# aurelienwaite/SparkNet

Measured on AMD Instinct MI355X. Metric: images/sec AlexNet training (227x227) at 1/2/4/8 MI355X; scaling efficiency, higher is better.
Workload: dtype bf16; 1 GPU; model=caffenet (bvlc_reference_caffenet / AlexNet), global_batch=256, per_gpu_batch=256, parallelism=dp1, algorithm=local SGD, tau=50, RCCL all-reduce weight averaging, hipgraph=True, streams=3, feed_group=2, fused_input_fold=True, fp8_layers=0, fp8_wgrad=False

## Files before the change

### sparknet_amd/ops/hip.py

```python
from __future__ import annotations

import contextlib
import ctypes as C
import dataclasses
import os
from typing import NamedTuple

import torch

from . import _lib
from ..utils import features
from .gemm import (EPI_BF16, EPI_F32, EPI_F32_ACC, ConvGeom, Dense, FlipW, Fp8Side, Im2col, colsum, fp8_side_output,
                   gemm, linear_dgrad, linear_fwd, linear_wgrad, side_bytes)
from .spec import POOL_MAX, ConvNdSpec, ConvSpec, PoolSpec

call = _lib.call
BF16 = torch.bfloat16
DGRAD_INPLACE_WEIGHTS = False


def _c(t: torch.Tensor) -> torch.Tensor:
    return t if t.is_contiguous() else t.contiguous()


# ... 1 lines not shown
    if t.is_contiguous():
        return t.shape[-1]
    if t.dim() != 4 or t.stride(-1) != 1:
        return 0
    N, H, W, Cc = t.shape
    ld = t.stride(2)
    if ld < Cc or t.stride(1) != W * ld or (N > 1 and t.stride(0) != H * W * ld):
        return 0
    return ld


def as_bf16(t: torch.Tensor | None) -> torch.Tensor | None:
    if t is None:
        return None
    t = _c(t)
    if t.dtype == BF16:
        return t
    if t.dtype != torch.float32:
        raise TypeError(f"GPU activations are bf16 or fp32, got {t.dtype}")
    out = torch.empty(t.shape, dtype=BF16, device=t.device)
    call("cast_f32_bf16", t, out, t.numel())
    return out


def _round8(n: int) -> int:
    return -(-n // 8) * 8



def _implicit_ok(s: ConvSpec) -> bool:
    return s.Cg % 8 == 0 and s.C % 8 == 0


def _unit_conv(s: ConvSpec) -> bool:
    return s.sh == 1 and s.sw == 1 and s.dh == 1 and s.dw == 1


def _wgrad_implicit_ok(s: ConvSpec) -> bool:
    return _implicit_ok(s) and s.Kg % 8 == 0


def _dgrad_flip_geom_ok(s: ConvSpec) -> bool:
    return _unit_conv(s) and _wgrad_implicit_ok(s)


def _plain_window(s: ConvSpec, r: int, p: int) -> bool:
    return s.groups == 1 and _unit_conv(s) and s.R == s.S == r and s.ph == s.pw == p


def _tile_rows_fit(s: ConvSpec, extra: int, lds_bytes: int) -> bool:
    return min(s.H, (191 + s.Q - 1) // s.Q + extra) * s.W * s.C * 2 <= lds_bytes


def _weight_kpad(w: torch.Tensor, s: ConvSpec) -> tuple[torch.Tensor, int]:
    kred = s.R * s.S * s.Cg
    kpad = _round8(kred)
    w2 = w.reshape(s.K, kred)
    if kpad == kred:
        return _c(w2), kpad
    out = torch.zeros((s.K, kpad), dtype=BF16, device=w.device)
    out[:, :kred].copy_(w2)
    return out, kpad


def _im2col(x: torch.Tensor, s: ConvSpec, g: int, kpad: int) -> torch.Tensor:
    M = s.N * s.P * s.Q
    col = torch.empty((M, kpad), dtype=BF16, device=x.device)
    call("im2col", x, col, s.N, s.H, s.W, s.C, s.P, s.Q, s.R, s.S, s.sh, s.sw, s.ph, s.pw, s.dh, s.dw,
         s.Cg, kpad, g * s.Cg)
    return col


def _geom(s: ConvSpec, ldx: int | None = None) -> ConvGeom:
    return ConvGeom(s.N, s.H, s.W, s.C if ldx is None else ldx, s.P, s.Q, s.R, s.S, s.sh, s.sw, s.ph, s.pw, s.dh, s.dw, s.Cg)


def _s2d_plan(s: ConvSpec):
    if _implicit_ok(s) or s.groups != 1 or s.sh != s.sw or s.dh != 1 or s.dw != 1:
        return None
    f = s.sh
    cp = s.C
    while (f * f * cp) % 8:
        cp += 1
    rf, sf = -(-s.R // f), -(-s.S // f)
    hs, ws = s.P + rf - 1, s.Q + sf - 1
    s2 = ConvSpec(s.N, hs, ws, f * f * cp, s.K, rf, sf, 1, 1, 0, 0, 1, 1, 1)
    assert s2.P == s.P and s2.Q == s.Q
    return f, cp, rf, sf, s2


def _s2d_input(x, s: ConvSpec, plan):
    f, cp, rf, sf, s2 = plan
    x2 = torch.empty((s.N, s2.H, s2.W, s2.C), dtype=BF16, device=x.device)
    call("s2d_input", x, x2, s.N, s.H, s.W, s.C, s2.H, s2.W, f, cp, s.ph, s.pw)
    return x2


def _s2d_cached(entry, x):
    return entry[2] if entry is not None and entry[:2] == (x.data_ptr(), x._version) else None


def _slice_ok(s: ConvSpec) -> bool:
    return s.groups == 1 and _wgrad_implicit_ok(s)


_MAX_PIX = 1 << 24


def _image_chunk(s: ConvSpec) -> int:
    per = max(s.H * s.W, s.P * s.Q, 1)
    plan = _s2d_plan(s)
    if plan is not None:
        per = max(per, plan[4].H * plan[4].W)
    return s.N if s.N * per < _MAX_PIX else max(1, (_MAX_PIX - 1) // per)


def conv_forward(x, w, b, s: ConvSpec, relu=False, ws=None, folded=None, out=None):
    nb = _image_chunk(s)
    if nb < s.N:
        y = out if out is not None else torch.empty((s.N, s.P, s.Q, s.K), dtype=BF16, device=x.device)
        for n0 in range(0, s.N, nb):
            n1 = min(s.N, n0 + nb)
            conv_forward(x[n0:n1], w, b, s.with_batch(n1 - n0), relu, None,
                         folded[n0:n1] if folded is not None else None, out=y[n0:n1])
        if ws is not None and folded is not None:
            ws.s2d_full = (x.data_ptr(), x._version, folded)
        return y
    ldx = chan_stride(x)
    if not (ldx and _slice_ok(s)):
        x, ldx = _c(x), s.C
    assert x.dtype == BF16 and w.dtype == BF16, (x.dtype, w.dtype)
    if out is not None:
        ldo = chan_stride(out)
        assert (out.is_contiguous() or _slice_ok(s)) and ldo and tuple(out.shape) == (s.N, s.P, s.Q, s.K) \
            and out.dtype == BF16, "conv output slice needs an ungrouped implicit conv and an NHWC channel-slice view"
    plan = _s2d_plan(s)
    if plan is not None:
        f, cp, rf, sf, s2 = plan
        w2 = ws.w2 if ws is not None else None
        if w2 is None:
            w2 = torch.empty((s.K, rf, sf, s2.C), dtype=BF16, device=x.device)
            call("s2d_weight", _c(w), w2, s.K, s.R, s.S, s.C, f, cp, rf, sf)
        else:
            assert tuple(w2.shape) == (s.K, rf, sf, s2.C) and w2.dtype == BF16 and w2.is_contiguous()
        x2 = folded if folded is not None else _s2d_input(x, s, plan)
        if ws is not None:
            ws.s2d = (x.data_ptr(), x._version, x2)
        return conv_forward(x2, w2, b, s2, relu, out=out)
    M = s.N * s.P * s.Q
    if out is not None:
        y, ldy = out, chan_stride(out)
    else:
        y, ldy = torch.empty((s.N, s.P, s.Q, s.K), dtype=BF16, device=x.device), s.K
    if ldx == s.C and ldy == s.K and x.is_contiguous() and packed3x3k64_ok(s):
        from . import gemm as G
        side = G._SIDE if _side_covers(y) else None
        if side is None or not side.e5m2:
            q = (None, None, None)
            if side is not None:
                q = (side.q.data_ptr() + (y.data_ptr() - side.base.data_ptr()) // 2, side.slot, side.part)
                side.launches += 1
            call("conv_packed3x3k64", x, _c(w), b, y, s.N, s.H, s.W, s.C, s.K, int(relu), *q)
            return y
    direct_io = ldx == s.C and ldy == s.K and x.is_contiguous() and not _side_covers(y)
    if direct_io and packed_conv_ok(s):
        call("conv_packed3x3", x, _c(w), b, y, s.N, s.H, s.W, s.C, s.K, int(relu))
        return y
    if direct_io and packed11_conv_ok(s):
        call("conv_packed1x1", x, _c(w), b, y, s.N, s.H, s.W, s.C, s.K, int(relu))
        return y
    if direct_io and packed44_conv_ok(s):
        call("conv_packed4x4", x, _c(w), b, y, s.N, s.H, s.W, s.C, s.K, int(relu))
        return y
    if direct_io and direct_conv_ok(s):
        call("conv3x3_direct", x, _c(w), b, None, y, s.N, s.H, s.W, s.C, s.K, s.ph, int(relu), 0)
        return y
    if direct_io and direct96_split_ok(s):
        wc = _c(w)
        for j in range(0, s.K, 96):
            call("conv3x3_direct", x, wc[j:j + 96], b[j:j + 96] if b is not None else None, None, y[..., j:],
                 s.N, s.H, s.W, s.C, 96, s.ph, int(relu), s.K)
        return y
    if direct_io and ldy == s.K and depthwise_ok(s) and _dw_io_ok(x, w, y):
        call("conv_dw_fwd", x, w, b, y, s.N, s.H, s.W, s.C, s.sh, s.sw, s.ph, s.pw, int(relu))
        return y
    if direct_io and ldy == s.K and grouped_ok(s) and _dw_io_ok(x, w, y):
        call(GROUPED_FWD, x, w, b, y, s.N, s.H, s.W, s.C, s.Cg, s.sh, s.sw, s.ph, s.pw, int(relu))
        return y
    if _implicit_ok(s):
        kred = s.R * s.S * s.Cg
        A = Im2col(x, _geom(s, ldx), kcontig=True, gstride=s.Cg)
        B = Dense(_c(w.reshape(s.K, kred)), kred, True, gstride=s.Kg * kred)
        gemm(M, s.Kg, kred, A, B, y, ldy, epi=EPI_BF16, groups=s.groups, c_gstride=s.Kg, bias=b, relu=relu)
        return y
    assert ldy == s.K, "explicit im2col path writes contiguous outputs"
    wp, kpad = _weight_kpad(w, s)
    y2 = y.view(M, s.K)
    for g in range(s.groups):
        col = _im2col(x, s, g, kpad)
        wg = wp[g * s.Kg:(g + 1) * s.Kg]
        bg = b[g * s.Kg:(g + 1) * s.Kg] if b is not None else None
        gemm(M, s.Kg, kpad, Dense(col, kpad, True), Dense(_c(wg), kpad, True), y2[:, g * s.Kg:], s.K,
             epi=EPI_BF16, bias=bg, relu=relu)
    return y


_DIRECT_C64 = features.enabled("conv_direct_c64")
_DIRECT_K96 = features.enabled("conv_direct_k96")


def direct_c64_ok(s: ConvSpec) -> bool:
    return _DIRECT_C64 and s.C == 64 and s.K == 64 and _plain_window(s, 3, 1)


def direct_conv_ok(s: ConvSpec) -> bool:
    return direct_c64_ok(s) or (_DIRECT_K96 and s.C == 48 and s.K == 96 and _plain_window(s, 3, 0))


_DIRECT96 = features.enabled("conv_direct96")


def direct96_split_ok(s: ConvSpec) -> bool:
    return _DIRECT96 and 0 < s.C <= 64 and s.C % 8 == 0 and s.K > 96 and s.K % 96 == 0 and _plain_window(s, 3, 1)


_PACKED11 = features.enabled("conv_packed11")


def packed11_conv_ok(s: ConvSpec) -> bool:
    return (_PACKED11 and 0 < s.C <= 64 and s.C % 8 == 0 and s.K == 64 and _plain_window(s, 1, 0)
            and _tile_rows_fit(s, 1, 36864))


_PACKED = features.enabled("conv_packed")


def packed_conv_ok(s: ConvSpec) -> bool:
    return (_PACKED and s.K == 96 and 0 < s.C <= 48 and s.C % 8 == 0 and _plain_window(s, 3, 0) and s.Q > 0
            and _tile_rows_fit(s, 3, 38400) and s.P * s.Q * 96 < 2 ** 31)


_PACKED44 = features.enabled("conv_packed44")


def packed44_conv_ok(s: ConvSpec) -> bool:
    return (_PACKED44 and s.K == 64 and s.C in (8, 16) and _plain_window(s, 4, 0) and s.Q > 0
            and _tile_rows_fit(s, 4, 22528) and s.P * s.Q * 64 < 2 ** 31)


_PACKED_K64 = features.enabled("conv_packed_k64")


def packed3x3k64_ok(s: ConvSpec) -> bool:
    return (_PACKED_K64 and s.K == 64 and s.C == 8 and _plain_window(s, 3, 0) and s.Q > 0
            and _tile_rows_fit(s, 3, 16384) and s.P * s.Q * 64 < 2 ** 31)


_DIRECT_FP8 = features.enabled("conv_direct_fp8")


def direct_fp8_ok(s: ConvSpec) -> bool:
    return _DIRECT_FP8 and direct_c64_ok(s)


def depthwise_ok(s: ConvSpec) -> bool:
    return (s.groups == s.C == s.K and s.C % 8 == 0 and s.R == 3 and s.S == 3 and s.dh == 1 and s.dw == 1
            and features.enabled("conv_depthwise"))


def _dw_io_ok(*tensors) -> bool:
    return all(t is None or (t.dtype == BF16 and t.is_contiguous() and t.data_ptr() % 16 == 0) for t in tensors)


def _dw_part(s: ConvSpec, device) -> tuple[torch.Tensor, int]:
    k = _lib.kernels()
    k.sn_conv_dw_part_floats.restype = C.c_longlong
    n = int(k.sn_conv_dw_part_floats(*(C.c_longlong(v) for v in (s.N, s.P, s.Q, s.C))))
    if n <= 0:
        raise ValueError(f"depthwise weight gradient: unsupported geometry {s}")
    return torch.empty(n, dtype=torch.float32, device=device), n


GROUPED_WIDTHS = (4, 8, 16)
_GROUPED_MAX_PIX = 1 << 30
GROUPED_FWD, GROUPED_WGRAD, GROUPED_DGRAD = "conv_grouped_fwd", "conv_grouped_wgrad", "conv_grouped_dgrad"


def grouped_ok(s: ConvSpec) -> bool:
    return (1 < s.Cg == s.Kg and s.Cg in GROUPED_WIDTHS and s.C % 16 == 0 and s.R == 3 and s.S == 3
            and s.dh == 1 and s.dw == 1 and s.sh in (1, 2) and s.sw in (1, 2)
            and max(s.N * s.H * s.W, s.N * s.P * s.Q) < _GROUPED_MAX_PIX and s.P > 0 and s.Q > 0
            and max(s.C, s.ph, s.pw) <= 1 << 20 and features.enabled("conv_grouped"))


def _grouped_part(s: ConvSpec, device) -> tuple[torch.Tensor, int]:
    k = _lib.kernels()
    k.sn_conv_grouped_part_floats.restype = C.c_longlong
    n = int(k.sn_conv_grouped_part_floats(*(C.c_longlong(v) for v in (s.N, s.P, s.Q, s.C, s.Cg))))
    if n <= 0:
        raise ValueError(f"grouped weight gradient: unsupported geometry {s}")
    return torch.empty(n, dtype=torch.float32, device=device), n


def _side_covers(t: torch.Tensor) -> bool:
    from . import gemm as G
    return G._SIDE is not None and G._SIDE.covers(t)


def dgrad_uses_flip(s: ConvSpec) -> bool:
    return _dgrad_flip_geom_ok(s) and not DGRAD_INPLACE_WEIGHTS


class Fp8Dgrad(NamedTuple):
    scales: object
    dy_slot: int
    wt_slot: int
    dy_side: object = None

    @property
    def dy_only(self) -> bool:
        return bool(getattr(self.dy_side, "only", False))


class Fp8Wgrad(NamedTuple):
    scales: object
    x_slot: int
    xq: torch.Tensor
    dy_slot: int


@dataclasses.dataclass
class ConvScratch:
    s2d: tuple | None = None
    s2d_full: tuple | None = None
    wt: torch.Tensor | None = None
    w2: torch.Tensor | None = None
    dw2: torch.Tensor | None = None
    fp8_dgrad: Fp8Dgrad | None = None
    fp8_wgrad: Fp8Wgrad | None = None
    fp8_dx_side: tuple | None = None
    fp8_dx_side_out: object = None

    def release(self) -> None:
        self.__init__()


class FlipBatch:

    def __init__(self, items, device):
        self.items = list(items)
        self.device = torch.device(device)
        self._build()

    def _ptrs(self):
        return [(w.data_ptr(), wt.data_ptr()) for w, wt, *_ in self.items]

    def _build(self):
        lib = _lib.kernels()
        lib.sn_flip_desc_size.restype = C.c_int
        size = lib.sn_flip_desc_size()
        buf = (C.c_char * (size * len(self.items)))()
        for i, (w, wt, G, Kg, R, S, Cg) in enumerate(self.items):
            assert w.is_contiguous() and wt.is_contiguous() and w.dtype == BF16 and wt.dtype == BF16
            assert w.numel() == wt.numel() == G * Kg * R * S * Cg < (1 << 31)
            lib.sn_flip_desc(C.byref(buf, i * size), C.c_void_p(w.data_ptr()), C.c_void_p(wt.data_ptr()),
                             *(C.c_longlong(v) for v in (G, Kg, R, S, Cg)))
        self.descs = torch.frombuffer(bytearray(buf), dtype=torch.uint8).to(self.device)
        self.max_tiles = max(G * R * S * -(-Kg // 64) * -(-Cg // 64) for _, _, G, Kg, R, S, Cg in self.items)
        self.ptrs = self._ptrs()

    def run(self) -> None:
        if self._ptrs() != self.ptrs:
            self._build()
        call("flip_weights_multi", self.descs, len(self.items), self.max_tiles)


def _pad_cols(t2: torch.Tensor, n: int) -> torch.Tensor:
    out = torch.zeros((t2.shape[0], n), dtype=t2.dtype, device=t2.device)
    out[:, :t2.shape[1]].copy_(t2)
    return out


def conv_backward(dy, x, w, s: ConvSpec, need_dx: bool, dw=None, db=None, gate=None, ws=None,
                  dw_acc=True, db_acc=True, dx_out=None):
    ws = ConvScratch() if ws is None else ws
    nb = _image_chunk(s)
    if dx_out is not None and need_dx and chan_stride(dx_out) != s.C and not (
            _dgrad_flip_geom_ok(s) and chan_stride(dx_out) and nb >= s.N
            and ws.fp8_dgrad is None and ws.fp8_dx_side is None):
        dx_out.copy_(conv_backward(dy, x, w, s, need_dx, dw, db, gate, ws, dw_acc, db_acc))
        return dx_out
    dx, side = dx_out if need_dx else None, None
    side_req, ws.fp8_dx_side = ws.fp8_dx_side, None
    if side_req is not None and need_dx and dx_out is None:
        dx = torch.empty((s.N, s.H, s.W, s.C), dtype=BF16, device=x.device)
        side = Fp8Side(dx, *side_req)
    with fp8_side_output(side) if side is not None else contextlib.nullcontext():
        if nb >= s.N:
            out = _conv_backward(dy, x, w, s, need_dx, dw, db, gate, ws, None, dw_acc, db_acc, dx)
        else:
            if dx is None and need_dx:
                dx = torch.empty((s.N, s.H, s.W, s.C), dtype=BF16, device=x.device)
            out = dx
            full = _s2d_cached(ws.s2d_full, x)
            dyq = _fp8_dyq(dy, ws)
            f8w = ws.fp8_wgrad
            for n0 in range(0, s.N, nb):
                n1 = min(s.N, n0 + nb)
                cws = ConvScratch(wt=ws.wt, fp8_dgrad=ws.fp8_dgrad,
                                  fp8_wgrad=f8w and f8w._replace(xq=f8w.xq[n0:n1]),
                                  s2d=full if full is None else (x[n0:n1].data_ptr(), x._version, full[n0:n1]))
                _conv_backward(dy[n0:n1], x[n0:n1], w, s.with_batch(n1 - n0), need_dx, dw, db,
                               gate[n0:n1] if gate is not None else None, cws,
                               None if dyq is None else dyq[n0:n1], dw_acc, db_acc, dx[n0:n1] if need_dx else None)
                dw_acc = db_acc = True
    ws.fp8_dx_side_out = side if out is dx else None
    return out


def _conv_backward(dy, x, w, s: ConvSpec, need_dx, dw, db, gate, ws: ConvScratch, dyq, dw_acc, db_acc, dx_out):
    kred = s.R * s.S * s.Cg
    plan = _s2d_plan(s) if s.Kg % 8 == 0 else None
    ldd, ldx = chan_stride(dy), chan_stride(x)
    if plan is not None or not _slice_ok(s) or not (ldd and ldx):
        dy, ldd, x, ldx = _c(dy), s.K, _c(x), s.C
    M = s.N * s.P * s.Q
    dy2 = dy.view(M, s.K) if ldd == s.K else dy
    fused_db = db is not None and dw is not None and (plan is not None or _wgrad_implicit_ok(s))
    f8w = ws.fp8_wgrad
    if (f8w is not None and dw is not None and plan is None and ldd == s.K and ldx == s.C
            and fp8_wgrad_ok(s) and f8w.xq.shape[0] == s.N):
        if dyq is None:
            dyq = _fp8_dyq(dy, ws)
        _conv_wgrad_fp8(dy2, dyq, s, M, kred, f8w, dw, db, dw_acc, db_acc, _dy_fp8_only(ws))
        dw, db, fused_db = None, None, False
    if (dw is not None or db is not None) and _dy_fp8_only(ws):
        _no_bf16_dy("a bf16 weight / bias gradient")
    _conv_wgrad(dy2, x, s, M, kred, plan, fused_db, dw, db, ws, dw_acc, db_acc, ldd, ldx)
    return _conv_dgrad(dy, x, w, s, M, gate, ws, dyq, ldd, ldx, dx_out) if need_dx else None


def _conv_wgrad(dy2, x, s, M, kred, plan, fused_db, dw, db, ws, dw_acc, db_acc, ldd, ldx):
    if ((dw is not None or db is not None) and plan is None and ldd == s.K and ldx == s.C and depthwise_ok(s)
            and _dw_io_ok(dy2, x)):
        part, n = _dw_part(s, x.device)
        call("conv_dw_wgrad", dy2, x, part, n, dw, 0 if dw is None else 1 + int(dw_acc),
             db, 0 if db is None else 1 + int(db_acc), s.N, s.H, s.W, s.C, s.sh, s.sw, s.ph, s.pw)
        return
    if dw is not None and plan is None and ldd == s.K and ldx == s.C and grouped_ok(s) and _dw_io_ok(dy2, x):
        if db is not None:
            colsum(dy2, db, accumulate=db_acc)
        part, n = _grouped_part(s, x.device)
        call(GROUPED_WGRAD, dy2, x, part, n, dw, int(dw_acc), s.N, s.H, s.W, s.C, s.Cg, s.sh, s.sw, s.ph, s.pw)
        return
    if db is not None and not fused_db:
        assert ldd == s.K
        colsum(dy2, db, accumulate=db_acc)
    if dw is not None and plan is not None:
        f, cp, rf, sf, s2 = plan
        x2 = _s2d_cached(ws.s2d, x)
        if x2 is None:
            x2 = _s2d_input(x, s, plan)
        k2 = rf * sf * s2.C
        keep = ws.dw2
        if keep is not None:
            assert not dw_acc, "a folded weight gradient left for the solver tail cannot accumulate"
            assert tuple(keep.shape) == (s.K, k2) and keep.dtype == torch.float32 and keep.is_contiguous()
        dw2 = keep if keep is not None else torch.empty((s.K, k2), dtype=torch.float32, device=x.device)
        gemm(s.K, k2, M, Dense(dy2, s.K, kcontig=False), Im2col(x2, _geom(s2), kcontig=False), dw2, k2,
             epi=EPI_F32, bias_grad=db if fused_db else None, bias_acc=db_acc)
        if keep is None:
            call("s2d_weight_grad", dw2, dw, s.K, s.R, s.S, s.C, f, cp, rf, sf, int(dw_acc))
        dw = None
    if dw is not None:
        if _wgrad_implicit_ok(s):
            A = Dense(dy2, ldd, kcontig=False, gstride=s.Kg)
            B = Im2col(x, _geom(s, ldx), kcontig=False, gstride=s.Cg)
            gemm(s.Kg, kred, M, A, B, dw, kred, epi=EPI_F32_ACC if dw_acc else EPI_F32, groups=s.groups,
                 c_gstride=s.Kg * kred, bias_grad=db if fused_db else None, bias_acc=db_acc)
        else:
            kpad = _round8(kred)
            kgp = _round8(s.Kg)
            dw2 = dw.view(s.K, kred)
            for g in range(s.groups):
                col = _im2col(x, s, g, kpad)
                dyg = dy2[:, g * s.Kg:(g + 1) * s.Kg]
                dyg = _c(dyg) if kgp == s.Kg else _pad_cols(dyg, kgp)
                tmp = torch.zeros((kgp, kpad), dtype=torch.float32, device=x.device)
                gemm(kgp, kpad, M, Dense(dyg, dyg.stride(0), False), Dense(col, kpad, False), tmp, kpad,
                     epi=EPI_F32)
                dwg = dw2[g * s.Kg:(g + 1) * s.Kg]
                (dwg.add_ if dw_acc else dwg.copy_)(tmp[:s.Kg, :kred])


FP8_WGRAD_BIAS = features.enabled("fp8_wgrad_bias")


def fp8_wgrad_ok(s: ConvSpec) -> bool:
    return _implicit_ok(s) and s.Kg % 16 == 0 and s.Cg % 16 == 0 and s.C % 16 == 0 and s.K % 16 == 0


def conv_dy_fp8_only_ok(layer, s: ConvSpec) -> bool:
    if layer.fp8_dgrad_slots is None or not fp8_dgrad_ok(s) or _s2d_plan(s) is not None:
        return False
    need_w = layer.param_grads_needed(0)
    need_b = layer.bias is not None and layer.param_grads_needed(1)
    if need_w and not (layer.fp8_wgrad and fp8_wgrad_ok(s)):
        return False
    return not need_b or (need_w and (s.R * s.S * s.Cg) % 16 == 0 and FP8_WGRAD_BIAS)


def _dy_fp8_only(ws: ConvScratch) -> bool:
    return ws.fp8_dgrad is not None and ws.fp8_dgrad.dy_only


def _no_bf16_dy(what: str):
    raise RuntimeError(f"conv backward: {what} would read the bf16 output gradient, which the max pooling "
                       "above stored only as fp8 (engine.fuse_fp8_quant fp8_dx_only; SN_FEATURES=fp8_dx_only=0)")


def _fp8_dyq(dy, ws: ConvScratch):
    f8, f8w = ws.fp8_dgrad, ws.fp8_wgrad
    if f8 is None and f8w is None:
        return None
    sc, idy, side = (f8.scales, f8.dy_slot, f8.dy_side) if f8 is not None else (f8w.scales, f8w.dy_slot, None)
    e5 = sc.is_e5m2(idy)
    dyq = side_bytes(side, dy, e5)
    if dyq is None and _dy_fp8_only(ws):
        _no_bf16_dy("quantising dy")
    return dyq if dyq is not None else quant_fp8(_c(dy), sc.slot(idy), e5m2=e5)


def _conv_wgrad_fp8(dy2, dyq, s, M, kred, f8w, dw, db, dw_acc, db_acc, dy_fp8_only=False):
    sc, ix, xq, idy = f8w
    fused_db = db is not None and kred % 16 == 0 and FP8_WGRAD_BIAS
    if db is not None and not fused_db:
        if dy_fp8_only:
            _no_bf16_dy("the exact bias gradient")
        colsum(dy2, db, accumulate=db_acc)
    A = Dense(dyq.view(M, s.K), s.K, kcontig=False, gstride=s.Kg)
    B = Im2col(xq, _geom(s), kcontig=False, gstride=s.Cg)
    gemm(s.Kg, kred, M, A, B, dw, kred, epi=EPI_F32_ACC if dw_acc else EPI_F32, groups=s.groups,
         c_gstride=s.Kg * kred, deq=(sc.deq(idy), sc.deq(ix), 2 if sc.is_e5m2(idy) else 1),
         bias_grad=db if fused_db else None, bias_acc=db_acc)


def _flipped(w, s, pre):
    if pre is not None:
        return pre
    wt = torch.empty((s.groups, s.Cg, s.R, s.S, s.Kg), dtype=BF16, device=w.device)
    call("flip_weights", _c(w), wt, s.groups, s.Kg, s.R, s.S, s.Cg)
    return wt


def _conv_dgrad(dy, x, w, s, M, gate, ws, dyq, ldd, ldx, dx_out):
    dx = dx_out if dx_out is not None else torch.empty((s.N, s.H, s.W, s.C), dtype=BF16, device=x.device)
    ldo = chan_stride(dx)
    if gate is not None and chan_stride(gate) != ldo:
        gate = _c(gate)
    flip = _dgrad_flip_geom_ok(s)
    fp8 = flip and ws.fp8_dgrad is not None and fp8_dgrad_ok(s) and ldd == s.K
    if _dy_fp8_only(ws) and not fp8:
        _no_bf16_dy("a bf16 data gradient")
    if (ldd == s.K and grouped_ok(s) and ws.fp8_dgrad is None and _dw_io_ok(dy, w, dx, gate)
            and not _side_covers(dx)):
        call(GROUPED_DGRAD, dy, w, gate, dx, s.N, s.H, s.W, s.C, s.Cg, s.sh, s.sw, s.ph, s.pw)
        return dx
    if flip:
        g2 = ConvGeom(s.N, s.P, s.Q, ldd, s.H, s.W, s.R, s.S, 1, 1, s.R - 1 - s.ph, s.S - 1 - s.pw, 1, 1, s.Kg)
        kr2 = s.R * s.S * s.Kg
        if fp8:
            return _conv_dgrad_fp8(dy, w, s, g2, kr2, gate, dx, ws, dyq)
        if (direct_c64_ok(s) and ldd == s.K and ldx == s.C and dy.is_contiguous() and dx.is_contiguous()
                and not DGRAD_INPLACE_WEIGHTS and not _side_covers(dx)):
            call("conv3x3_direct", dy, _flipped(w, s, ws.wt), None, _c(gate) if gate is not None else None, dx,
                 s.N, s.H, s.W, 64, 64, 1, 0, 0)
            return dx
        A = Im2col(dy, g2, kcontig=True, gstride=s.Kg)
        if DGRAD_INPLACE_WEIGHTS:
            B = FlipW(_c(w), s.Kg, s.R, s.S, s.Cg)
        else:
            B = Dense(_flipped(w, s, ws.wt).view(s.C, kr2), kr2, True, gstride=s.Cg * kr2)
        gemm(s.N * s.H * s.W, s.Cg, kr2, A, B, dx, ldo, epi=EPI_BF16, groups=s.groups, c_gstride=s.Cg, gate=gate)
        return dx
    if ldd == s.K and depthwise_ok(s) and _dw_io_ok(dy, w, dx, gate) and not _side_covers(dx):
        call("conv_dw_dgrad", dy, w, gate, dx, s.N, s.H, s.W, s.C, s.sh, s.sw, s.ph, s.pw)
        return dx
    assert ldd == s.K
    dy2 = dy.view(M, s.K)
    wp, kpad = _weight_kpad(w, s)
    kgp = _round8(s.Kg)
    for g in range(s.groups):
        dyg = dy2[:, g * s.Kg:(g + 1) * s.Kg]
        dyg = _c(dyg) if kgp == s.Kg else _pad_cols(dyg, kgp)
        wg = wp[g * s.Kg:(g + 1) * s.Kg]
        if kgp != s.Kg:
            wg = torch.cat([wg, torch.zeros((kgp - s.Kg, kpad), dtype=BF16, device=x.device)])
        dcol = torch.empty((M, kpad), dtype=torch.float32, device=x.device)
        gemm(M, kpad, kgp, Dense(dyg, dyg.stride(0), True), Dense(_c(wg), kpad, False), dcol, kpad, epi=EPI_F32)
        call("col2im", dcol, dx, s.N, s.H, s.W, s.C, s.P, s.Q, s.R, s.S, s.sh, s.sw, s.ph, s.pw, s.dh, s.dw,
             s.Cg, kpad, g * s.Cg)
    if gate is not None:
        dx = relu_backward(dx, gate)
        if dx_out is not None:
            dx_out.copy_(dx)
            dx = dx_out
    return dx


def fp8_dgrad_ok(s: ConvSpec) -> bool:
    return dgrad_uses_flip(s) and s.Kg % 16 == 0 and s.C % 8 == 0


def _conv_dgrad_fp8(dy, w, s, g2, kr2, gate, dx, ws: ConvScratch, dyq):
    sc, idy, iwt, _ = ws.fp8_dgrad
    wt = _flipped(w, s, ws.wt)
    e5 = sc.is_e5m2(idy)
    if dyq is None:
        dyq = _fp8_dyq(dy, ws)
    wtq = quant_fp8(wt, sc.slot(iwt))
    if direct_fp8_ok(s) and not e5 and dx.is_contiguous() and not _side_covers(dx):
        call("conv3x3_fp8", _c(dyq), wtq, sc.deq(idy), sc.deq(iwt), None, _c(gate) if gate is not None else None, dx,
             s.N, s.H, s.W, 0)
        return dx
    A = Im2col(dyq, g2, kcontig=True, gstride=s.Kg)
    B = Dense(wtq.view(s.C, kr2), kr2, True, gstride=s.Cg * kr2)
    gemm(s.N * s.H * s.W, s.Cg, kr2, A, B, dx, s.C, epi=EPI_BF16, groups=s.groups, c_gstride=s.Cg,
         gate=_c(gate) if gate is not None else None, deq=(sc.deq(idy), sc.deq(iwt), 2 if e5 else 1))
    return dx



def linear_forward(x2, w, b, relu=False, dropout=None):
    return linear_fwd(_c(x2), _c(w), b, relu, dropout=dropout)


def linear_backward(dy2, x2, w, need_dx, dw=None, db=None, gate=None, dw_acc=True, db_acc=True, gate_scale=1.0):
    dy2 = _c(dy2)
    if dw is not None:
        if not linear_wgrad(dy2, _c(x2), dw, accumulate=dw_acc, db=db, db_acc=db_acc) and db is not None:
            colsum(dy2, db, accumulate=db_acc)
    elif db is not None:
        colsum(dy2, db, accumulate=db_acc)
    if not need_dx:
        return None
    return linear_dgrad(dy2, _c(w), gate=gate.reshape(x2.shape) if gate is not None else None,
                        gate_scale=gate_scale)


def linear_backward_sgd(dy2, x2, w, need_dx, sgd, db=None, gate=None, db_acc=True, gate_scale=1.0):
    dy2, x2 = _c(dy2), _c(x2)
    dx = None
    if need_dx:
        dx = linear_dgrad(dy2, _c(w), gate=gate.reshape(x2.shape) if gate is not None else None,
                          gate_scale=gate_scale)
    from .gemm import linear_wgrad_sgd
    if not linear_wgrad_sgd(dy2, x2, sgd, db, db_acc) and db is not None:
        colsum(dy2, db, accumulate=db_acc)
    return dx



def _nd_dims(s: ConvNdSpec):
    v = list(s.ins) + list(s.outs) + list(s.ks) + list(s.st) + list(s.pd)
    return (C.c_int * len(v))(*v)


def _nd_dt(t: torch.Tensor) -> int:
    assert t.dtype in (BF16, torch.float32), t.dtype
    return int(t.dtype == torch.float32)


def _nd_col(x, s: ConvNdSpec, g: int) -> torch.Tensor:
    ld = _round8(s.Cg * s.T)
    col = torch.empty((s.num * s.P, ld), dtype=BF16, device=x.device)
    call("im2col_nd", x, col, s.nd, s.num, s.C, s.Cg, g * s.Cg, ld, _nd_dims(s), _nd_dt(x), 0)
    return col


def _nd_chan_cl(t, s: ConvNdSpec, chans: int, g: int, per: int) -> torch.Tensor:
    from . import layers_hip as lh
    if s.groups == 1:
        return lh.transpose(t, s.num, chans, s.P).view(s.num * s.P, chans)
    tmp = torch.empty((s.num, per, s.P), dtype=t.dtype, device=t.device)
    lh.axis_copy(t, tmp, s.num, chans, per, s.P, g * per, 0, per)
    return lh.transpose(tmp, s.num, per, s.P).view(s.num * s.P, per)


def conv_nd_forward(x, w, b, s: ConvNdSpec):
    from . import layers_hip as lh
    x = _c(x)
    CT = s.Cg * s.T
    y = torch.empty((s.num, s.K, s.P), dtype=BF16, device=x.device)
    for g in range(s.groups):
        col = _nd_col(x, s, g)
        wg = torch.zeros((s.Kg, col.shape[1]), dtype=BF16, device=x.device)
        wg[:, :CT] = w[g * s.Kg:(g + 1) * s.Kg].reshape(s.Kg, CT)
        bg = b[g * s.Kg:(g + 1) * s.Kg].float().contiguous() if b is not None else None
        yc = linear_fwd(col, wg, bg)
        if s.groups == 1:
            y = lh.transpose(yc, s.num, s.P, s.Kg, out_shape=(s.num, s.K, s.P))
        else:
            lh.axis_copy(lh.transpose(yc, s.num, s.P, s.Kg), y, s.num, s.Kg, s.K, s.P, 0, g * s.Kg, s.Kg)
    return y.view((s.num, s.K) + s.outs)


def conv_nd_backward(dy, x, w, s: ConvNdSpec, need_dx: bool, dw=None, db=None):
    dy = _c(dy).to(BF16)
    if x is not None:
        x = _c(x)
    assert x is not None or dw is None, "the weight gradient needs the input"
    CT = s.Cg * s.T
    dx = torch.empty((s.num, s.C) + s.ins, dtype=dy.dtype, device=dy.device) if need_dx else None
    for g in range(s.groups):
        dyc = _nd_chan_cl(dy, s, s.K, g, s.Kg)
        if dw is not None:
            col = _nd_col(x, s, g)
            dwg = dw.view(s.K, CT)[g * s.Kg:(g + 1) * s.Kg]
            dbg = db[g * s.Kg:(g + 1) * s.Kg] if db is not None else None
            if not linear_wgrad(dyc, col[:, :CT], dwg, accumulate=True, db=dbg, db_acc=True) and dbg is not None:
                colsum(dyc, dbg, accumulate=True)
        elif db is not None:
            colsum(dyc, db[g * s.Kg:(g + 1) * s.Kg], accumulate=True)
        if need_dx:
            wg = w[g * s.Kg:(g + 1) * s.Kg].reshape(s.Kg, CT).contiguous()
            dcol = linear_dgrad(dyc, wg)
            call("col2im_nd", dcol, dx, s.nd, s.num, s.C, s.Cg, g * s.Cg, dcol.stride(0), _nd_dims(s), 0,
                 _nd_dt(dx), 0)
    return dx



def _pool_args(s: PoolSpec):
    return (s.N, s.H, s.W, s.C, s.P, s.Q, s.kh, s.kw, s.sh, s.sw, s.ph, s.pw, s.method)


_MAX_ELEMS = 1 << 31


def _pool_images(s: PoolSpec) -> int:
    per = s.H * s.W * s.C
    return s.N if s.N * per < _MAX_ELEMS else max(1, (_MAX_ELEMS - 1) // per)


def pool_side_ok(s: PoolSpec, backward: bool) -> bool:
    if s.C % 8:
        return False
    if not backward:
        return s.method == POOL_MAX and s.kh == s.kw and s.kh in (2, 3)
    nh, nw = -(-s.kh // s.sh), -(-s.kw // s.sw)
    return not (s.kh == 3 and s.kw == 3 and s.sh == 2 and s.sw == 2) and nh == nw and 1 <= nh <= 3


def _side_args(side, t, n0, n1):
    if side is None:
        return (None, None, None, 0)
    return (side.q[n0:n1], side.slot, side.part, int(side.e5m2))


def pool_forward_mask(x, s: PoolSpec, gate: bool = False, side=None):
    x = _c(x)
    if side is not None:
        assert pool_side_ok(s, False) and tuple(side.base.shape) == (s.N, s.P, s.Q, s.C)
        y = side.base
    else:
        y = torch.empty((s.N, s.P, s.Q, s.C), dtype=BF16, device=x.device)
    mask = torch.empty((s.N, s.P, s.Q, s.C), dtype=torch.uint8, device=x.device) if s.method == POOL_MAX else None
    nb = _pool_images(s)
    for n0 in range(0, s.N, nb):
        n1 = min(s.N, n0 + nb)
        call("pool_fwd", x[n0:n1], y[n0:n1], mask[n0:n1] if mask is not None else None,
             *_pool_args(dataclasses.replace(s, N=n1 - n0)), int(gate and s.method == POOL_MAX),
             *_side_args(side, y, n0, n1))
    if side is not None:
        side.launches += 1
        side.finish()
    return y, mask


def pool_forward(x, s: PoolSpec):
    return pool_forward_mask(x, s)[0]


def pool_backward(dy, x, s: PoolSpec, mask=None, y=None, gate=False, side=None, side_only=False):
    if side_only:
        assert side is not None and s.method == POOL_MAX
        side.only = True
    if side is not None:
        assert pool_side_ok(s, True) and not (gate and s.method != POOL_MAX)
        assert tuple(side.base.shape) == (s.N, s.H, s.W, s.C)
        dx = side.base
    else:
        dx = torch.empty((s.N, s.H, s.W, s.C), dtype=BF16, device=dy.device)
    if s.method == POOL_MAX and mask is None:
        _, mask = pool_forward_mask(x, s, gate)
    dy = _c(dy)
    nb = _pool_images(s)
    for n0 in range(0, s.N, nb):
        n1 = min(s.N, n0 + nb)
        call("pool_bwd", dy[n0:n1], mask[n0:n1] if mask is not None else None, None if side_only else dx[n0:n1],
             *_pool_args(dataclasses.replace(s, N=n1 - n0)), *_side_args(side, dx, n0, n1))
    if side is not None:
        side.launches += 1
        side.finish()
    if gate and s.method != POOL_MAX:
        dx = relu_backward(dx, x)
    return dx


def pool_lrn_eligible(s: PoolSpec, size: int, within: bool) -> bool:
    if s.method != POOL_MAX or within or (s.kh, s.kw, s.sh, s.sw) != (3, 3, 2, 2) or s.C % 8 or size not in (3, 5, 7, 9):
        return False
    if s.ph >= 3 or s.pw >= 3 or s.N * s.H * s.W * s.C >= 1 << 32:
        return False
    fn = _lib.kernels().sn_pool_lrn_supported
    fn.restype = C.c_int
    return bool(fn(*(C.c_longlong(v) for v in (s.N, s.H, s.W, s.C, s.P, s.Q, s.ph, s.pw, size))))


def pool_lrn_forward(x, s: PoolSpec, gate: bool, size: int, alpha: float, beta: float, k: float):
    x = _c(x)
    pooled = torch.empty((s.N, s.P, s.Q, s.C), dtype=BF16, device=x.device)
    mask = torch.empty((s.N, s.P, s.Q, s.C), dtype=torch.uint8, device=x.device)
    y = torch.empty_like(pooled)
    call("pool_lrn_fwd", x, pooled, mask, y, s.N, s.H, s.W, s.C, s.P, s.Q, s.ph, s.pw, int(gate), int(size),
         float(alpha), float(beta), float(k))
    return pooled, mask, y


def lrn_pool_backward(dy, pooled, mask, s: PoolSpec, size: int, alpha: float, beta: float, k: float):
    dx = torch.empty((s.N, s.H, s.W, s.C), dtype=BF16, device=dy.device)
    call("lrn_pool_bwd", _c(pooled), _c(dy), mask, dx, s.N, s.H, s.W, s.C, s.P, s.Q, s.ph, s.pw, int(size),
         float(alpha), float(beta), float(k))
    return dx


def pool_lrn_rev_eligible(s: PoolSpec, size: int, within: bool) -> bool:
    if s.method != POOL_MAX or within or (s.kh, s.kw, s.sh, s.sw) != (3, 3, 2, 2) or s.C % 8 or size not in (3, 5, 7, 9):
        return False
    if s.ph >= 3 or s.pw >= 3 or s.N * s.H * s.W * s.C >= 1 << 32 or s.C > 8192:
        return False
    if 2 * (s.P - 1) - s.ph >= s.H or 2 * (s.Q - 1) - s.pw >= s.W:
        return False
    return (s.H + s.ph + 1) // 2 <= s.P + 1 and (s.W + s.pw + 1) // 2 <= s.Q + 1


def pool_lrn_backward_rev(dy, mask, x, s: PoolSpec, size: int, alpha: float, beta: float, k: float,
                          gate: bool = False):
    x = _c(x)
    assert tuple(x.shape) == (s.N, s.H, s.W, s.C) and tuple(mask.shape) == (s.N, s.P, s.Q, s.C)
    dx = torch.empty_like(x)
    call("pool_lrn_bwd_rev", _c(dy), _c(mask), x, dx, s.N, s.H, s.W, s.C, s.P, s.Q, s.ph, s.pw, int(size),
         float(alpha), float(beta), float(k), int(gate))
    return dx


def lrn_forward(x, size, alpha, beta, k, within=False):
    x = _c(x)
    N, H, W, Cc = x.shape
    y = torch.empty_like(x)
    if within:
        call("lrn_within_fwd", x, y, None, N, H, W, Cc, size, float(alpha), float(beta))
    else:
        call("lrn_across_fwd", x, y, N, H, W, Cc, size, float(alpha), float(beta), float(k))
    return y


def lrn_backward(dy, x, size, alpha, beta, k, within=False, y=None, gate=False):
    x, dy = _c(x), _c(dy)
    N, H, W, Cc = x.shape
    dx = torch.empty_like(x)
    if within:
        sbuf = torch.empty(x.shape, dtype=torch.float32, device=x.device)
        u = torch.empty(x.shape, dtype=torch.float32, device=x.device)
        call("lrn_within_bwd", x, dy, sbuf, u, dx, N, H, W, Cc, size, float(alpha), float(beta))
        if gate:
            dx = relu_backward(dx, x)
    else:
        call("lrn_across_bwd", x, dy, dx, N, H, W, Cc, size, float(alpha), float(beta), float(k), int(gate))
    return dx
# ... 394 lines not shown
```

### sparknet_amd/utils/features.py

```python
from __future__ import annotations

import os

DEFAULTS = {
    "fuse_pool_lrn": True,
    "fuse_lrn_pool_bwd": True,
    "zero_copy_concat": True,
    "fuse_dropout": True,
    "fuse_fp8_quant": True,
    "fuse_bn_scale": True,
    "branch_depfree": True,
    "fuse_splitk": False,
    "fuse_loss_head": True,
    "loss_head_without_tail": False,
    "solver_tail": True,
    "solver_tail_flips": False,
    "conv_direct_c64": True,
    "conv_direct_k96": True,
    "conv_direct96": True,
    "conv_packed": True,
    "conv_packed44": True,
    "conv_packed11": False,
    "conv_packed_k64": True,
    "conv_direct_fp8": True,
    "conv_depthwise": True,
    "conv_grouped": True,
    "fp8_wgrad_bias": True,
    "fp8_side_frag": True,
    "fp8_dx_only": True,
}

_cache: tuple[str, dict] = ("", {})


def _parsed() -> dict:
    global _cache
    raw = os.environ.get("SN_FEATURES", "")
    if raw != _cache[0]:
        out = {}
        for item in filter(None, (p.strip() for p in raw.split(","))):
            name, _, val = item.partition("=")
            if name not in DEFAULTS:
                raise ValueError(f"SN_FEATURES: unknown switch {name!r} (known: {', '.join(sorted(DEFAULTS))})")
            out[name] = val.strip().lower() not in ("0", "false", "off", "no")
        _cache = (raw, out)
    return _cache[1]


def enabled(name: str) -> bool:
    if name not in DEFAULTS:
        raise KeyError(name)
    return _parsed().get(name, DEFAULTS[name])
```

Before: 121,600 images/sec.

## Add warp-specialized LDS patch kernel for conv2 5x5 grouped data gradient

Adds a dedicated HIP kernel for the 5x5, stride-1, pad-2 grouped convolution data gradient with Kg=128 and Cg=48, which matches AlexNet conv2. Producer waves stage a haloed input-gradient patch and a ring of flipped-weight tap slices in LDS, while consumer waves run MFMA bf16 over all 25 taps with the ReLU gate fused. This replaces the im2col-plus-GEMM path and is meant to avoid materializing the im2col matrix and to reuse patch data across taps. It is enabled by default through a new feature switch, but it adds a large amount of hand-written code that has correctness risk.

```diff
diff --git a/csrc/kernels/conv_patch.hip b/csrc/kernels/conv_patch.hip
--- /dev/null
+++ b/csrc/kernels/conv_patch.hip
@@ -0,0 +1,241 @@
+#include "common.h"
+#include "conv_patch_plan.h"
+
+namespace {
+
+using namespace sn_patch;
+
+struct Args {
+  Plan p;
+  FDiv fw, fpw;
+  uint32_t items;
+  float gate_scale;
+};
+
+
+SN_DEV bf16x8_t lds_frag(const unsigned char* a) {
+  return __builtin_bit_cast(bf16x8_t, *reinterpret_cast<const u32x4*>(a));
+}
+
+struct Item {
+  int n, g, h0, rows;
+};
+
+SN_DEV Item item_of(const Plan& p, uint32_t it) {
+  const uint32_t b1 = it / (uint32_t)p.G, n = b1 / (uint32_t)p.nb;
+  Item r;
+  r.g = (int)(it - b1 * p.G);
+  r.n = (int)n;
+  r.h0 = (int)(b1 - n * p.nb) * p.bh;
+  r.rows = min(p.bh, p.H - r.h0);
+  return r;
+}
+
+SN_DEV uint32_t fetch(const bf16_t* __restrict__ dy, const bf16_t* __restrict__ wt, const Args& a, const Item& it,
+                      int tid, u32x4* pv, u32x4* w0, u32x4* w1) {
+  const Plan& p = a.p;
+  const int kc = tid & 15, npix = (it.rows + HALO) * p.pw;
+  const bf16_t* src = dy + (long long)it.n * p.H * p.W * p.ldd + (long long)it.g * KG;
+  uint32_t inside = 0;
+  int pr = (int)udiv((uint32_t)(tid >> 4), a.fpw), pc = (tid >> 4) - pr * p.pw;
+#pragma unroll
+  for (int u = 0; u < PPT; ++u) {
+    const int r = it.h0 - 2 + pr, c = pc - 2;
+    const bool ok = ((tid >> 4) + 16 * u < npix) & (r >= 0) & (r < p.H) & (c >= 0) & (c < p.W);
+    const int rc = min(max(r, 0), p.H - 1), cc = min(max(c, 0), p.W - 1);
+    pv[u] = *reinterpret_cast<const u32x4*>(src + (uint32_t)((rc * p.W + cc) * (int)p.ldd + kc * 8));
+    inside |= (uint32_t)ok << u;
+    pc += 16;
+    if (pc >= p.pw) { pc -= p.pw; ++pr; }
+    if (pc >= p.pw) { pc -= p.pw; ++pr; }
+  }
+  const bf16_t* wsrc = wt + (long long)it.g * CG * (TAPS * KG);
+  const uint32_t woff = (uint32_t)((tid >> 4) * (TAPS * KG) + kc * 8);
+#pragma unroll
+  for (int j = 0; j < 3; ++j) {
+    w0[j] = *reinterpret_cast<const u32x4*>(wsrc + woff + j * 16 * (TAPS * KG));
+    w1[j] = *reinterpret_cast<const u32x4*>(wsrc + woff + j * 16 * (TAPS * KG) + KG);
+  }
+  return inside;
+}
+
+__global__ void __launch_bounds__(128 * NWAVE) conv_patch_dgrad_k(const bf16_t* __restrict__ dy,
+                                                                  const bf16_t* __restrict__ wt,
+                                                                  const bf16_t* __restrict__ gate,
+                                                                  bf16_t* __restrict__ dx, const Args a) {
+  extern __shared__ __attribute__((aligned(16))) unsigned char sm[];
+  unsigned char* const patch = sm + RING * WSLOT;
+  const Plan& p = a.p;
+  const int lane = threadIdx.x & 63, wave = threadIdx.x >> 6;
+  const int tid = threadIdx.x & (64 * NWAVE - 1);
+  const int q = lane >> 4, kc = tid & 15;
+  unsigned char* const wdst = sm + (kc & 1) * WHALF + (tid >> 4) * HPIX + (kc >> 1) * 16;
+  uint32_t item = blockIdx.x;
+  Item cur = item_of(p, item);
+
+  if (wave >= NWAVE) {
+    unsigned char* const pdst = patch + (kc & 1) * p.half + (tid >> 4) * HPIX + (kc >> 1) * 16;
+    u32x4 pv[PPT], w0[3], w1[3];
+    uint32_t inside = fetch(dy, wt, a, cur, tid, pv, w0, w1);
+    for (;;) {
+      const int npix = (cur.rows + HALO) * p.pw;
+#pragma unroll
+      for (int u = 0; u < PPT; ++u)
+        if ((tid >> 4) + 16 * u < npix)
+          *reinterpret_cast<u32x4*>(pdst + u * 16 * HPIX) = (inside >> u) & 1 ? pv[u] : u32x4{0u, 0u, 0u, 0u};
+#pragma unroll
+      for (int j = 0; j < 3; ++j) {
+        *reinterpret_cast<u32x4*>(wdst + j * 16 * HPIX) = w0[j];
+        *reinterpret_cast<u32x4*>(wdst + WSLOT + j * 16 * HPIX) = w1[j];
+      }
+      const uint32_t next = item + gridDim.x;
+      const bool has_next = next < a.items;
+      if (has_next) cur = item_of(p, next);
+      __syncthreads();
+      if (has_next) inside = fetch(dy, wt, a, cur, tid, pv, w0, w1);
+      for (int t = 0; t < TAPS; ++t) __syncthreads();
+      if (!has_next) return;
+      item = next;
+    }
+  }
+
+  const unsigned char* const bbase = sm + (q & 1) * WHALF + (lane & 15) * HPIX + (q >> 1) * 16;
+  u32x4 wv[3];
+  for (;;) {
+    const unsigned char* abase[4];
+    int opix[4];
+    const int mlim = cur.rows * p.W;
+#pragma unroll
+    for (int f = 0; f < 4; ++f) {
+      const int m = wave * MWAVE + f * 16 + (lane & 15);
+      const int mm = m < mlim ? m : 0;
+      const int lr = (int)udiv((uint32_t)mm, a.fw), w = mm - lr * p.W;
+      abase[f] = patch + (q & 1) * p.half + (lr * p.pw + w) * HPIX + (q >> 1) * 16;
+      opix[f] = m < mlim ? (cur.h0 + lr) * p.W + w : -1;
+    }
+    const bf16_t* wsrc = wt + ((long long)cur.g * CG + (tid >> 4)) * (TAPS * KG) + kc * 8;
+
+    f32x4 acc[4][3];
+#pragma unroll
+    for (int f = 0; f < 4; ++f)
+#pragma unroll
+      for (int i = 0; i < 3; ++i) acc[f][i] = f32x4{0.f, 0.f, 0.f, 0.f};
+
+    __syncthreads();
+
+    bf16x8_t fa[4], fb[3];
+#pragma unroll
+    for (int f = 0; f < 4; ++f) fa[f] = lds_frag(abase[f]);
+#pragma unroll
+    for (int i = 0; i < 3; ++i) fb[i] = lds_frag(bbase + i * 16 * HPIX);
+
+    int tr = 0, ts = 0, toff = 0, slot = 0;
+    for (int t = 0; t < TAPS; ++t) {
+      const bool more = t + 2 < TAPS;
+      if (more) {
+#pragma unroll
+        for (int j = 0; j < 3; ++j)
+          wv[j] = *reinterpret_cast<const u32x4*>(wsrc + (long long)j * 16 * (TAPS * KG) + (t + 2) * KG);
+      }
+      int nr = tr, ns = ts + 1;
+      if (ns == RS) {
+        ns = 0;
+        ++nr;
+      }
+      if (nr == RS) {
+        nr = tr;
+        ns = ts;
+      }
+      const int noff = (nr * p.pw + ns) * HPIX;
+      const int nslot = slot + 1 == RING ? 0 : slot + 1;
+#pragma unroll
+      for (int s = 0; s < 4; ++s) {
+        bf16x8_t na[4], nb[3];
+        const int ao = s < 3 ? toff + 32 * (s + 1) : noff;
+        const int bo = s < 3 ? slot * WSLOT + 32 * (s + 1) : nslot * WSLOT;
+#pragma unroll
+        for (int f = 0; f < 4; ++f) na[f] = lds_frag(abase[f] + ao);
+#pragma unroll
+        for (int i = 0; i < 3; ++i) nb[i] = lds_frag(bbase + bo + i * 16 * HPIX);
+        __builtin_amdgcn_s_setprio(1);
+#pragma unroll
+        for (int i = 0; i < 3; ++i)
+#pragma unroll
+          for (int f = 0; f < 4; ++f)
+            acc[f][i] = __builtin_amdgcn_mfma_f32_16x16x32_bf16(fb[i], fa[f], acc[f][i], 0, 0, 0);
+        __builtin_amdgcn_s_setprio(0);
+#pragma unroll
+        for (int f = 0; f < 4; ++f) fa[f] = na[f];
+#pragma unroll
+        for (int i = 0; i < 3; ++i) fb[i] = nb[i];
+      }
+      if (more) {
+        const int wslot = nslot + 1 == RING ? 0 : nslot + 1;
+#pragma unroll
+        for (int j = 0; j < 3; ++j) *reinterpret_cast<u32x4*>(wdst + wslot * WSLOT + j * 16 * HPIX) = wv[j];
+      }
+      __syncthreads();
+      tr = nr;
+      ts = ns;
+      toff = noff;
+      slot = nslot;
+    }
+
+#pragma unroll
+    for (int f = 0; f < 4; ++f) {
+      if (opix[f] < 0) continue;
+      const long long e0 = ((long long)cur.n * p.H * p.W + opix[f]) * p.ldo + (long long)cur.g * CG + 4 * q;
+#pragma unroll
+      for (int i = 0; i < 3; ++i) {
+        const long long e = e0 + 16 * i;
+        float o[4] = {acc[f][i][0], acc[f][i][1], acc[f][i][2], acc[f][i][3]};
+        if (gate) {
+          const uint2 u = *reinterpret_cast<const uint2*>(gate + e);
+          const float gv[4] = {__uint_as_float(u.x << 16), __uint_as_float(u.x & 0xffff0000u),
+                               __uint_as_float(u.y << 16), __uint_as_float(u.y & 0xffff0000u)};
+#pragma unroll
+          for (int r = 0; r < 4; ++r) o[r] = gv[r] > 0.f ? o[r] * a.gate_scale : 0.f;
+        }
+        *reinterpret_cast<uint2*>(dx + e) = make_uint2(pack2(o[0], o[1]), pack2(o[2], o[3]));
+      }
+    }
+    item += gridDim.x;
+    if (item >= a.items) return;
+    cur = item_of(p, item);
+  }
+}
+
+inline bool al16(const void* p) { return (reinterpret_cast<uintptr_t>(p) & 15) == 0; }
+
+}
+
+extern "C" {
+
+int sn_conv_patch_plan(long long N, long long H, long long W, long long G, long long ldd, long long ldo,
+                       long long* bands, long long* band_rows, long long* lds_bytes) {
+  Plan p;
+  const bool ok = make_plan(N, H, W, G, ldd, ldo, p);
+  if (bands) *bands = ok ? p.nb : 0;
+  if (band_rows) *band_rows = ok ? p.bh : 0;
+  if (lds_bytes) *lds_bytes = ok ? (long long)p.lds : 0;
+  return ok ? 0 : 3;
+}
+
+int sn_conv_patch_dgrad(const bf16_t* dy, const bf16_t* wt, const bf16_t* gate, bf16_t* dx, long long N, long long H,
+                        long long W, long long G, long long ldd, long long ldo, float gate_scale, long long max_blocks,
+                        hipStream_t st) {
+  Args a;
+  if (!make_plan(N, H, W, G, ldd, ldo, a.p)) return 3;
+  if (!dy || !wt || !dx || !al16(dy) || !al16(wt) || !al16(gate) || !al16(dx)) return 2;
+  a.fw = make_fdiv((uint32_t)a.p.W);
+  a.fpw = make_fdiv((uint32_t)a.p.pw);
+  a.gate_scale = gate_scale;
+  a.items = a.p.items;
+  if (max_blocks < 0) return 3;
+  const long long cap = max_blocks ? max_blocks : sn_cu_count();
+  const unsigned grid = (unsigned)(a.items < cap ? a.items : cap);
+  hipLaunchKernelGGL(conv_patch_dgrad_k, dim3(grid), dim3(128 * NWAVE), a.p.lds, st, dy, wt, gate, dx, a);
+  return SN_CHECK_LAUNCH();
+}
+
+}
diff --git a/csrc/kernels/conv_patch_plan.h b/csrc/kernels/conv_patch_plan.h
--- /dev/null
+++ b/csrc/kernels/conv_patch_plan.h
@@ -0,0 +1,50 @@
+#pragma once
+#include <stddef.h>
+
+namespace sn_patch {
+
+constexpr int KG = 128;
+constexpr int CG = 48;
+constexpr int RS = 5, TAPS = 25;
+constexpr int HALO = RS - 1;
+constexpr int NWAVE = 4, MWAVE = 64, MBLK = NWAVE * MWAVE;
+constexpr int HPIX = 144;
+constexpr int WHALF = CG * HPIX;
+constexpr int WSLOT = 2 * WHALF;
+constexpr int RING = 3;
+constexpr int LDS_MAX = 160 * 1024;
+constexpr int PPT = 27;
+
+struct Plan {
+  int N, H, W, G;
+  int bh, nb;
+  int pw;
+  int half;
+  long long ldd, ldo;
+  unsigned items;
+  size_t lds;
+};
+
+inline int patch_half(int bh, int pw) { return ((bh + HALO) * pw * HPIX + 255) & ~255; }
+
+inline bool make_plan(long long N, long long H, long long W, long long G, long long ldd, long long ldo, Plan& p) {
+  if (N < 1 || H < 1 || W < 8 || G < 1 || W > MBLK || H > (1 << 20) || G > (1 << 12)) return false;
+  if (ldd < G * KG || ldo < G * CG || ldd > (1 << 20) || ldo > (1 << 20) || ldd % 8 != 0 || ldo % 4 != 0) return false;
+  if (N * H * W >= (1LL << 30) || H * W * ldd >= (1LL << 30)) return false;
+  const int pw = (int)W + HALO;
+  int bh = MBLK / (int)W;
+  if (bh > H) bh = (int)H;
+  while (bh >= 1 && (RING * WSLOT + 2 * patch_half(bh, pw) > LDS_MAX || (bh + HALO) * pw > 16 * PPT)) --bh;
+  if (bh < 1) return false;
+  const int nb = ((int)H + bh - 1) / bh;
+  bh = ((int)H + nb - 1) / nb;
+  if (N * G * nb >= (1LL << 31)) return false;
+  p.N = (int)N; p.H = (int)H; p.W = (int)W; p.G = (int)G;
+  p.bh = bh; p.nb = nb; p.pw = pw; p.half = patch_half(bh, pw);
+  p.ldd = ldd; p.ldo = ldo;
+  p.items = (unsigned)(N * G * nb);
+  p.lds = (size_t)RING * WSLOT + 2 * (size_t)p.half;
+  return true;
+}
+
+}
diff --git a/sparknet_amd/ops/hip.py b/sparknet_amd/ops/hip.py
--- a/sparknet_amd/ops/hip.py
+++ b/sparknet_amd/ops/hip.py
@@ -327,6 +327,16 @@
     return torch.empty(n, dtype=torch.float32, device=device), n
 
 
+PATCH_DGRAD = "conv_patch_dgrad"
+PATCH_MIN_ROWS, PATCH_MAX_COLS = 8, 32
+
+
+def patch_dgrad_ok(s: ConvSpec) -> bool:
+    return (s.R == 5 and s.S == 5 and _unit_conv(s) and s.ph == 2 and s.pw == 2 and s.Kg == 128 and s.Cg == 48
+            and PATCH_MIN_ROWS <= s.H and PATCH_MIN_ROWS <= s.W <= PATCH_MAX_COLS
+            and s.N * s.H * s.W < _GROUPED_MAX_PIX and features.enabled("conv_patch"))
+
+
 def _side_covers(t: torch.Tensor) -> bool:
     from . import gemm as G
     return G._SIDE is not None and G._SIDE.covers(t)
@@ -601,6 +611,10 @@
             call("conv3x3_direct", dy, _flipped(w, s, ws.wt), None, _c(gate) if gate is not None else None, dx,
                  s.N, s.H, s.W, 64, 64, 1, 0, 0)
             return dx
+        if (patch_dgrad_ok(s) and ldd == s.K and ldo == s.C and not DGRAD_INPLACE_WEIGHTS
+                and _dw_io_ok(dy, dx, gate) and not _side_covers(dx)):
+            call(PATCH_DGRAD, dy, _flipped(w, s, ws.wt), gate, dx, s.N, s.H, s.W, s.groups, ldd, ldo, 1.0, 0)
+            return dx
         A = Im2col(dy, g2, kcontig=True, gstride=s.Kg)
         if DGRAD_INPLACE_WEIGHTS:
             B = FlipW(_c(w), s.Kg, s.R, s.S, s.Cg)
diff --git a/sparknet_amd/utils/features.py b/sparknet_amd/utils/features.py
--- a/sparknet_amd/utils/features.py
+++ b/sparknet_amd/utils/features.py
@@ -25,6 +25,7 @@
     "conv_direct_fp8": True,
     "conv_depthwise": True,
     "conv_grouped": True,
+    "conv_patch": True,
     "fp8_wgrad_bias": True,
     "fp8_side_frag": True,
     "fp8_dx_only": True,
```

Result: faster. 123,200 images/sec, median of 6 (+1.4%).
